# YzM1a0/MuDPT

Measured on AMD Instinct MI355X. Metric: images/sec fwd+bwd ViT-B/16 MuDPT, higher is better.
Workload: dtype bf16; 1 GPU; MuDPT ViT-B/16 fwd+bwd+SGD, batch 256/GPU, 11 class prompts, n_ctx 4, depth 12, synthetic 224x224 N(0,1) images, random-init frozen CLIP (BASELINE configs[1]); global_batch=256, parallelism=dp1

## Files before the change

### mudpt_amd/csrc/gemm_pp.hip

```cpp
#include <hip/hip_ext.h>

#include <type_traits>

#include "kernels.h"

namespace mudpt {

using lptr_t = __attribute__((address_space(3))) void*;

#define VMCNT(n) asm volatile("s_waitcnt vmcnt(" #n ")" ::: "memory")
typedef __attribute__((ext_vector_type(4))) unsigned int u32x4;

template <int N>
__device__ inline void vmcnt() {
    static_assert(N >= 0 && N <= 63, "vmcnt immediate is 6 bits");
    asm volatile("s_waitcnt vmcnt(%0)" ::"n"(N) : "memory");
}

constexpr int EPI_GELU_SPLIT = 100;
constexpr int EPI_GELU_SPLIT8 = 101;
constexpr int EPI_GELU_Q8 = 102;
constexpr int EPI_GELU_BWD_Q8 = 103;

template <typename T, int EPI, bool F8 = false, int ST = 0, int LD = 0, int ABL = 0>
__global__ __launch_bounds__(512) void gemm_pp_kernel(GemmArgs p, int ntn, int ntiles, int rem_half) {
    using elem = typename T::elem;
    using vec8 = typename T::vec8;
    constexpr int STAGE = 65536, BOFF = 32768;
    extern __shared__ __attribute__((aligned(16))) char smem[];

    const int tid = threadIdx.x, lane = tid & 63;
    const int w = __builtin_amdgcn_readfirstlane(tid >> 6);
    const int wr = w >> 2, wc = w & 3;
    const int frow = lane & 15, fq = lane >> 4;

    const int nkt1 = p.K >> 6;
    const int nkt = nkt1 + (p.lo_mode == LO_NONE ? 0 : (F8 ? nkt1 >> 1 : nkt1));
    const int G = gridDim.x;
    const int my_full = rem_half ? ntiles / G : (ntiles - (int)blockIdx.x + G - 1) / G;
    const bool has_half = rem_half && (int)blockIdx.x < 2 * rem_half;
    const int total = (my_full + (has_half ? 1 : 0)) * nkt;

    const auto rsA = __builtin_amdgcn_make_buffer_rsrc(const_cast<void*>(p.A), 0, (int)((size_t)p.M * p.lda * 2 < 0xffffffffull ? (size_t)p.M * p.lda * 2 : 0xffffffffull), 0x00020000);
    const auto rsB = __builtin_amdgcn_make_buffer_rsrc(const_cast<void*>(p.B), 0, (int)((size_t)p.N * p.ldb * 2 < 0xffffffffull ? (size_t)p.N * p.ldb * 2 : 0xffffffffull), 0x00020000);
    const auto rsA2 = __builtin_amdgcn_make_buffer_rsrc(const_cast<void*>(p.A_lo ? p.A_lo : p.A), 0, (int)((size_t)p.M * p.lda * 2 < 0xffffffffull ? (size_t)p.M * p.lda * 2 : 0xffffffffull), 0x00020000);
    const auto rsB2 = __builtin_amdgcn_make_buffer_rsrc(const_cast<void*>(F8 ? p.B8 : p.B), 0, (int)((size_t)p.N * p.ldb * 2 < 0xffffffffull ? (size_t)p.N * p.ldb * 2 : 0xffffffffull), 0x00020000);

    static_assert(EPI == EPI_STORE || EPI == EPI_GELU || EPI == EPI_GELU_SPLIT || EPI == EPI_GELU_SPLIT8 || EPI == EPI_GELU_BWD || EPI == EPI_STORE_F32 ||
                  EPI == EPI_GELU_Q8 || EPI == EPI_GELU_BWD_Q8, "epilogue not built for gemm_pp");
    constexpr bool GELU = (EPI == EPI_GELU || EPI == EPI_GELU_SPLIT || EPI == EPI_GELU_SPLIT8 || EPI == EPI_GELU_Q8);
    constexpr int OOB = (int)0x80000000;
    constexpr bool OUT_F32 = (EPI == EPI_STORE_F32);
    constexpr bool NAT = OUT_F32;
    constexpr int NST = (EPI == EPI_STORE || EPI == EPI_GELU_BWD || EPI == EPI_GELU_BWD_Q8) ? 16 : (EPI == EPI_GELU_SPLIT ? 48 : (EPI == EPI_GELU_SPLIT8 ? 40 : (EPI == EPI_GELU_Q8 ? 24 : 32)));
    const auto rsOut0 = __builtin_amdgcn_make_buffer_rsrc(p.out0, 0, p.M * p.ldo0 * (OUT_F32 ? 4 : (EPI == EPI_GELU_Q8 ? 1 : 2)), 0x00020000);
    const auto rsOut1 = __builtin_amdgcn_make_buffer_rsrc(p.out1, 0, GELU ? p.M * p.ldo1 * 2 : 0, 0x00020000);
    const auto rsOut1Lo = __builtin_amdgcn_make_buffer_rsrc(p.out1_lo, 0, (EPI == EPI_GELU_SPLIT || EPI == EPI_GELU_SPLIT8) ? p.M * p.ldo1 * 2 : 0, 0x00020000);
    const auto rsAux = __builtin_amdgcn_make_buffer_rsrc(const_cast<void*>(p.aux), 0, EPI == EPI_GELU_BWD ? p.M * p.ldaux * 2 : (EPI == EPI_GELU_BWD_Q8 ? p.M * p.ldaux : 0), 0x00020000);
    const auto rsBias = __builtin_amdgcn_make_buffer_rsrc(const_cast<float*>(p.bias), 0, p.bias ? p.N * 4 : 0, 0x00020000);
    bool epi_pending = false;

    int grp[4][2];
#pragma unroll
    for (int q = 0; q < 2; ++q) {
        const int k = 2 * w + q;
        grp[0][q] = k < 8 ? k : k + 8;
        grp[3][q] = k < 8 ? k + 8 : k + 16;
        grp[1][q] = NAT ? (k >> 2) * 8 + (k & 3) : 2 * k;
        grp[2][q] = NAT ? (k >> 2) * 8 + (k & 3) + 4 : 2 * k + 1;
    }
    const int srow = lane >> 3, sslot = lane & 7;
    int lane_off[4][2];
#pragma unroll
    for (int u = 0; u < 4; ++u)
#pragma unroll
        for (int q = 0; q < 2; ++q) {
            const bool isA = (u == 0 || u == 3);
            const int row = grp[u][q] * 8 + srow;
            const int f = (isA || NAT) ? (row & 7) : ((row & 3) | (((row >> 4) & 1) << 2));
            lane_off[u][q] = (row * (isA ? p.lda : p.ldb) + ((sslot ^ f) << 3)) * 2;
        }

    const int gn_knob = (p.flags >> 8) & 0xff;
    const int GN = gn_knob > 0 ? gn_knob : (ntn >= 12 ? 6 : (ntn >= 6 && ntn % 3 == 0 ? 3 : ntn));
    const int ntm = ntiles / ntn;
    auto tile_mn = [&](int tile, int& tm, int& tn) {
        const int tpg = ntm * GN, full = ntn / GN, ng = tile / tpg;
        if (ng < full) {
            const int rem = tile - ng * tpg;
            tm = rem / GN;
            tn = ng * GN + (rem - tm * GN);
        } else {
            const int wl = ntn - full * GN, rem = tile - full * tpg;
            tm = rem / wl;
            tn = full * GN + (rem - tm * wl);
        }
    };
    auto item_tile = [&](int it, int& tm, int& tn, int& h) {
        if (it < my_full) {
            tile_mn(xcd_remap((int)blockIdx.x + it * G, ntiles), tm, tn);
            h = 0;
        } else {
            h = (int)blockIdx.x >= rem_half ? 1 : 0;
            tile_mn(xcd_remap(my_full * G + (int)blockIdx.x - h * rem_half, ntiles), tm, tn);
        }
    };
    int n_kt = 0, n_it = 0, n_baseA = 0, n_baseB = 0, n_soff = 0;
    bool n_second = false;
    bool n_half = false;
    auto set_next_item = [&](int it) {
        int tm, tn, h;
        item_tile(it, tm, tn, h);
        n_half = it >= my_full;
        n_baseA = (tm * 256 + (n_half ? h * 128 - (w >= 4 ? 64 : 0) : 0)) * p.lda * 2;
        n_baseB = tn * 256 * p.ldb * 2;
    };
    auto advance_next = [&]() {
        n_soff += 128;
        if (++n_kt == nkt) {
            n_kt = 0; n_soff = 0; n_second = false;
            if ((++n_it) * nkt < total) set_next_item(n_it);
        } else if (n_kt == nkt1) {
            n_soff = 0; n_second = true;
        }
    };
    auto issue = [&](int u, int stage) {
        if constexpr (ABL & 2) return;
        const bool isA = (u == 0 || u == 3);
        const int base = isA ? n_baseA : n_baseB;
        char* dst = smem + stage * STAGE + (isA ? 0 : BOFF);
#pragma unroll
        for (int q = 0; q < 2; ++q)
            __builtin_amdgcn_raw_ptr_buffer_load_lds(isA ? (n_second ? rsA2 : rsA) : (n_second ? rsB2 : rsB), (lptr_t)(dst + grp[u][q] * 1024), 16, lane_off[u][q] + base, n_soff, 0, 0);
    };

    const int sw = frow & 7;
    const int c0 = (fq ^ sw) << 4;
    const int c8 = ((2 * fq) ^ sw) << 4;
    int ca = c0, cb = c0 ^ 64;
    const int a_base = (wr * 128 + frow) * 128;
    const int b_base = BOFF + (NAT ? wc * 64 + frow : wc * 64 + (frow >> 2) * 16 + (frow & 3)) * 128;
    constexpr int BJ = NAT ? 2048 : 512;

    f32x4 acc[8][4];
#pragma unroll
    for (int i = 0; i < 8; ++i)
#pragma unroll
        for (int j = 0; j < 4; ++j) acc[i][j] = f32x4{0.f, 0.f, 0.f, 0.f};

    if (total > 0) {
        set_next_item(0);
        issue(0, 0); issue(1, 0); issue(2, 0);
        if (!n_half) issue(3, 0);
        advance_next();
    }
    VMCNT(0);
    __builtin_amdgcn_s_barrier();
    if (wr == 1) __builtin_amdgcn_s_barrier();

    typedef __attribute__((ext_vector_type(4))) int i32x4;
    i32x8 af[4], bf[4];
    if constexpr (ABL & 1) {
#pragma unroll
        for (int i = 0; i < 4; ++i) { af[i] = i32x8{lane, 1, 2, 3, 4, 5, 6, 7} * 0x3c003c00; bf[i] = i32x8{7, 6, 5, 4, 3, 2, 1, lane} * 0x3c003c00; }
    }
    auto half = [](const i32x8& v, int ks) -> vec8 {
        return __builtin_bit_cast(vec8, ks ? __builtin_shufflevector(v, v, 4, 5, 6, 7) : __builtin_shufflevector(v, v, 0, 1, 2, 3));
    };
    int c_it = 0;

    auto mfma_quadrant = [&](auto f8tag, int i0, int j0) {
        __builtin_amdgcn_sched_barrier(0);
        __builtin_amdgcn_s_setprio(1);
        if constexpr (decltype(f8tag)::value) {
#pragma unroll
            for (int i = 0; i < 4; ++i)
#pragma unroll
                for (int j = 0; j < 2; ++j)
                    acc[i0 + i][j0 + j] = __builtin_amdgcn_mfma_scale_f32_16x16x128_f8f6f4(bf[j0 + j], af[i], acc[i0 + i][j0 + j], 0, 0, 0, p.b8_scale, 0, LO8_SCALE_E8M0);
        } else {
#pragma unroll
            for (int ks = 0; ks < 2; ++ks)
#pragma unroll
                for (int i = 0; i < 4; ++i)
#pragma unroll
                    for (int j = 0; j < 2; ++j) acc[i0 + i][j0 + j] = T::mfma16(half(bf[j0 + j], ks), half(af[i], ks), acc[i0 + i][j0 + j]);
        }
        __builtin_amdgcn_s_setprio(0);
        __builtin_amdgcn_sched_barrier(0);
    };
    auto read_a = [&](const char* st, int i0) {
        if constexpr (ABL & 1) return;
#pragma unroll
        for (int i = 0; i < 4; ++i)
            af[i] = __builtin_shufflevector(*(const i32x4*)(st + a_base + (i0 + i) * 2048 + ca), *(const i32x4*)(st + a_base + (i0 + i) * 2048 + cb), 0, 1, 2, 3, 4, 5, 6, 7);
    };
    auto read_b = [&](const char* st, int j0) {
        if constexpr (ABL & 1) return;
#pragma unroll
        for (int j = j0; j < j0 + 2; ++j)
            bf[j] = __builtin_shufflevector(*(const i32x4*)(st + b_base + j * BJ + ca), *(const i32x4*)(st + b_base + j * BJ + cb), 0, 1, 2, 3, 4, 5, 6, 7);
    };
    auto epilogue = [&]() {
            int tm, tn, h;
            const bool c_half = c_it >= my_full;
            item_tile(c_it++, tm, tn, h);
            const int ni = c_half ? 4 : 8;
            const int n = tn * 256 + wc * 64 + (NAT ? fq * 4 : fq * 16);
            f32x4 bias4[4];
#pragma unroll
            for (int j = 0; j < 4; ++j)
                bias4[j] = p.bias ? __builtin_bit_cast(f32x4, __builtin_amdgcn_raw_buffer_load_b128(rsBias, (n + (NAT ? 16 : 4) * j) * 4, 0, 0)) : f32x4{0.f, 0.f, 0.f, 0.f};
            const int m_base = tm * 256 + (c_half ? h * 128 + wr * 64 : wr * 128) + frow;
            auto row_off = [&](int i, int ld, int esz, int col) { return (col < p.N ? (m_base * ld + col) * esz : OOB) + i * (16 * ld * esz); };
#pragma unroll
            for (int i = 0; i < 8; ++i)
#pragma unroll
                for (int j = 0; j < 4; ++j) acc[i][j] += bias4[j];
            if constexpr (EPI == EPI_GELU_BWD) {
                vec8 u[8][2];
#pragma unroll
                for (int i = 0; i < 8; ++i) {
                    const int off = i < ni ? row_off(i, p.ldaux, 2, n) : OOB;
                    u[i][0] = __builtin_bit_cast(vec8, __builtin_amdgcn_raw_buffer_load_b128(rsAux, off, 0, LD));
                    u[i][1] = __builtin_bit_cast(vec8, __builtin_amdgcn_raw_buffer_load_b128(rsAux, off, 16, LD));
                }
#pragma unroll
                for (int i = 0; i < 8; ++i)
#pragma unroll
                    for (int j = 0; j < 4; ++j)
#pragma unroll
                        for (int c = 0; c < 4; ++c) acc[i][j][c] *= quick_gelu_grad((float)u[i][j >> 1][4 * (j & 1) + c]);
            }
            if constexpr (EPI == EPI_GELU_BWD_Q8) {
                u32x4 q[8];
#pragma unroll
                for (int i = 0; i < 8; ++i) q[i] = __builtin_amdgcn_raw_buffer_load_b128(rsAux, i < ni ? row_off(i, p.ldaux, 1, n) : OOB, 0, LD);
#pragma unroll
                for (int i = 0; i < 8; ++i)
#pragma unroll
                    for (int j = 0; j < 4; ++j)
#pragma unroll
                        for (int c = 0; c < 4; ++c) acc[i][j][c] *= gelu_grad_from_q8(q[i][j], c);
            }
            __builtin_amdgcn_sched_barrier(0);
#pragma unroll
            for (int i = 0; i < 8; ++i) {
                if (i < ni) {
                if constexpr (OUT_F32) {
#pragma unroll
                    for (int j = 0; j < 4; ++j) __builtin_amdgcn_raw_buffer_store_b128(__builtin_bit_cast(u32x4, acc[i][j]), rsOut0, row_off(i, p.ldo0, 4, n + 16 * j), 0, ST);
                } else {
                    vec8 o0, o1;
                    if constexpr (EPI == EPI_GELU_Q8) {
                        u32x4 q;
#pragma unroll
                        for (int j = 0; j < 4; ++j) q[j] = gelu_grad_q8x4(acc[i][j][0], acc[i][j][1], acc[i][j][2], acc[i][j][3]);
                        __builtin_amdgcn_raw_buffer_store_b128(q, rsOut0, row_off(i, p.ldo0, 1, n), 0, ST);
                    } else {
#pragma unroll
                        for (int c = 0; c < 4; ++c) {
                            o0[c] = round_to<elem>(acc[i][0][c]); o0[4 + c] = round_to<elem>(acc[i][1][c]);
                            o1[c] = round_to<elem>(acc[i][2][c]); o1[4 + c] = round_to<elem>(acc[i][3][c]);
                        }
                        const int off = row_off(i, p.ldo0, 2, n);
                        __builtin_amdgcn_raw_buffer_store_b128(__builtin_bit_cast(u32x4, o0), rsOut0, off, 0, ST);
                        __builtin_amdgcn_raw_buffer_store_b128(__builtin_bit_cast(u32x4, o1), rsOut0, off, 16, ST);
                    }
                    if constexpr (EPI == EPI_GELU || EPI == EPI_GELU_Q8) {
#pragma unroll
                        for (int c = 0; c < 4; ++c) {
                            o0[c] = round_to<elem>(quick_gelu(acc[i][0][c])); o0[4 + c] = round_to<elem>(quick_gelu(acc[i][1][c]));
                            o1[c] = round_to<elem>(quick_gelu(acc[i][2][c])); o1[4 + c] = round_to<elem>(quick_gelu(acc[i][3][c]));
                        }
                        const int off1 = row_off(i, p.ldo1, 2, n);
                        __builtin_amdgcn_raw_buffer_store_b128(__builtin_bit_cast(u32x4, o0), rsOut1, off1, 0, ST);
                        __builtin_amdgcn_raw_buffer_store_b128(__builtin_bit_cast(u32x4, o1), rsOut1, off1, 16, ST);
                    }
                    if constexpr (EPI == EPI_GELU_SPLIT8) {
                        u32x4 l8;
                        float rem[4];
#pragma unroll
                        for (int j = 0; j < 4; ++j) {
#pragma unroll
                            for (int c = 0; c < 4; ++c) {
                                elem hv;
                                rem[c] = split_rem(quick_gelu(acc[i][j][c]), hv);
                                if (j < 2) o0[4 * j + c] = hv; else o1[4 * (j - 2) + c] = hv;
                            }
                            l8[j] = pack_lo8(rem[0], rem[1], rem[2], rem[3]);
                        }
                        const int off1 = row_off(i, p.ldo1, 2, n);
                        __builtin_amdgcn_raw_buffer_store_b128(__builtin_bit_cast(u32x4, o0), rsOut1, off1, 0, ST);
                        __builtin_amdgcn_raw_buffer_store_b128(__builtin_bit_cast(u32x4, o1), rsOut1, off1, 16, ST);
                        __builtin_amdgcn_raw_buffer_store_b128(l8, rsOut1Lo, (n < p.N ? m_base * p.ldo1 * 2 + n : OOB) + i * (32 * p.ldo1), 0, ST);
                    }
                    if constexpr (EPI == EPI_GELU_SPLIT) {
                        vec8 l0, l1;
#pragma unroll
                        for (int c = 0; c < 4; ++c) {
                            elem hv, lv;
                            split_hi_lo(quick_gelu(acc[i][0][c]), hv, lv); o0[c] = hv; l0[c] = lv;
                            split_hi_lo(quick_gelu(acc[i][1][c]), hv, lv); o0[4 + c] = hv; l0[4 + c] = lv;
                            split_hi_lo(quick_gelu(acc[i][2][c]), hv, lv); o1[c] = hv; l1[c] = lv;
                            split_hi_lo(quick_gelu(acc[i][3][c]), hv, lv); o1[4 + c] = hv; l1[4 + c] = lv;
                        }
                        const int off1 = row_off(i, p.ldo1, 2, n);
                        __builtin_amdgcn_raw_buffer_store_b128(__builtin_bit_cast(u32x4, o0), rsOut1, off1, 0, ST);
                        __builtin_amdgcn_raw_buffer_store_b128(__builtin_bit_cast(u32x4, o1), rsOut1, off1, 16, ST);
                        __builtin_amdgcn_raw_buffer_store_b128(__builtin_bit_cast(u32x4, l0), rsOut1Lo, off1, 0, ST);
                        __builtin_amdgcn_raw_buffer_store_b128(__builtin_bit_cast(u32x4, l1), rsOut1Lo, off1, 16, ST);
                    }
                }
                }
#pragma unroll
                for (int j = 0; j < 4; ++j) acc[i][j] = f32x4{0.f, 0.f, 0.f, 0.f};
            }
            epi_pending = true;
    };

    int s = 0;
    auto full_step = [&](auto f8tag) {
        constexpr bool F8S = decltype(f8tag)::value;
        const int cur = s & 1;
        const char* st = smem + cur * STAGE;
        const bool nxt = s + 1 < total;
        ca = F8S ? c8 : c0;
        cb = F8S ? (c8 ^ 16) : (c0 ^ 64);
        read_a(st, 0);
        read_b(st, 0);
        if (nxt) {
            issue(0, cur ^ 1);
            if (epi_pending) vmcnt<NST + 4>(); else vmcnt<4>();
        } else {
            if (epi_pending) vmcnt<NST + 2>(); else vmcnt<2>();
        }
        __builtin_amdgcn_s_barrier();
        mfma_quadrant(f8tag, 0, 0);
        __builtin_amdgcn_s_barrier();
        read_b(st, 2);
        if (nxt) {
            issue(1, cur ^ 1);
            if (epi_pending) vmcnt<NST + 4>(); else vmcnt<4>();
        } else {
            if (epi_pending) vmcnt<NST>(); else vmcnt<0>();
        }
        epi_pending = false;
        __builtin_amdgcn_s_barrier();
        mfma_quadrant(f8tag, 0, 2);
        __builtin_amdgcn_s_barrier();
        read_a(st, 4);
        if (nxt) issue(2, cur ^ 1);
        __builtin_amdgcn_s_barrier();
        mfma_quadrant(f8tag, 4, 2);
        __builtin_amdgcn_s_barrier();
        if (nxt) {
            if (!n_half) { issue(3, cur ^ 1); advance_next(); VMCNT(4); } else { advance_next(); VMCNT(2); }
        }
        __builtin_amdgcn_s_barrier();
        mfma_quadrant(f8tag, 4, 0);
        __builtin_amdgcn_s_barrier();
        ++s;
    };
    auto half_step = [&](auto f8tag) {
        constexpr bool F8S = decltype(f8tag)::value;
        const int cur = s & 1;
        const char* st = smem + cur * STAGE;
        const bool nxt = s + 1 < total;
        ca = F8S ? c8 : c0;
        cb = F8S ? (c8 ^ 16) : (c0 ^ 64);
        read_a(st, 0);
        read_b(st, 0);
        if (nxt) {
            issue(0, cur ^ 1);
            issue(1, cur ^ 1);
            if (epi_pending) vmcnt<NST + 4>(); else vmcnt<4>();
        } else {
            if (epi_pending) vmcnt<NST>(); else vmcnt<0>();
        }
        __builtin_amdgcn_s_barrier();
        mfma_quadrant(f8tag, 0, 0);
        __builtin_amdgcn_s_barrier();
        read_b(st, 2);
        if (nxt) { issue(2, cur ^ 1); advance_next(); VMCNT(2); }
        epi_pending = false;
        __builtin_amdgcn_s_barrier();
        mfma_quadrant(f8tag, 0, 2);
        __builtin_amdgcn_s_barrier();
        ++s;
    };
    const int nkt2 = nkt - nkt1;
    for (int it = 0; it < my_full; ++it) {
        if constexpr (F8) {
            for (int k = 0; k < nkt1; ++k) full_step(std::false_type{});
            for (int k = 0; k < nkt2; ++k) full_step(std::true_type{});
        } else {
            for (int k = 0; k < nkt; ++k) full_step(std::false_type{});
        }
        epilogue();
    }
    if (has_half) {
        if constexpr (F8) {
            for (int k = 0; k < nkt1; ++k) half_step(std::false_type{});
            for (int k = 0; k < nkt2; ++k) half_step(std::true_type{});
        } else {
            for (int k = 0; k < nkt; ++k) half_step(std::false_type{});
        }
        epilogue();
    }
    if (wr == 0) __builtin_amdgcn_s_barrier();
}

template <typename T, int EPI, bool F8 = false, int ST = 0, int LD = 0, int ABL = 0>
static int launch_pp(const GemmArgs& a, hipStream_t s, const GemmOpts& o) {
    constexpr int lds = 2 * 65536;
    constexpr auto kern = gemm_pp_kernel<T, EPI, F8, ST, LD, ABL>;
    const int dev = current_device(), ncu = device_cus(dev);
    if (ncu <= 0) return MUDPT_ERR_HIP;
    if (int e = lds_limit_once<kern>(dev, lds)) return e;
    const int ntm = (a.M + 255) / 256, ntn = (a.N + 255) / 256, ntiles = ntm * ntn;
    int grid = ntiles < ncu ? (2 * ntiles <= ncu ? 2 * ntiles : ntiles) : ncu;
    if (a.flags & 2) grid = ntiles < ncu ? ntiles : ncu;
    const int rem = ntiles % grid, rem_half = (rem > 0 && 2 * rem <= grid && !(a.flags & 2)) ? rem : 0;
    if (o.ev_start && o.ev_stop) {
        hipExtLaunchKernelGGL(kern, dim3(grid), dim3(512), lds, s, o.ev_start, o.ev_stop, 0, a, ntn, ntiles, rem_half);
    } else {
        hipLaunchKernelGGL(kern, dim3(grid), dim3(512), lds, s, a, ntn, ntiles, rem_half);
    }
    HIP_TRY(hipGetLastError());
    return MUDPT_OK;
}

template <typename T>
static int launch_pp_t(int epi, const GemmArgs& a, hipStream_t s, const GemmOpts& o) {
    if constexpr (T::id == DT_F16) {
        if (a.lo_mode == LO_F8) {
            switch (epi) {
                case EPI_STORE: return launch_pp<T, EPI_STORE, true>(a, s, o);
                case EPI_GELU:
                    if (!a.out1_lo) return launch_pp<T, EPI_GELU, true>(a, s, o);
                    return a.out1_lo_mode == LO_F8 ? launch_pp<T, EPI_GELU_SPLIT8, true>(a, s, o) : launch_pp<T, EPI_GELU_SPLIT, true>(a, s, o);
                case EPI_STORE_F32: return launch_pp<T, EPI_STORE_F32, true>(a, s, o);
            }
            set_error("gemm_pp: epilogue %d is not built with the e4m3 second pass", epi);
            return MUDPT_ERR_ARG;
        }
    }
    if constexpr (T::id == DT_BF16) {
        if (epi == EPI_STORE && (a.flags & 0x30)) {
            switch ((a.flags >> 4) & 3) {
                case 1: return launch_pp<T, EPI_STORE, false, 0, 0, 1>(a, s, o);
                case 2: return launch_pp<T, EPI_STORE, false, 0, 0, 2>(a, s, o);
                default: return launch_pp<T, EPI_STORE, false, 0, 0, 3>(a, s, o);
            }
        }
    }
    switch (epi) {
        case EPI_STORE: return launch_pp<T, EPI_STORE>(a, s, o);
        case EPI_GELU:
            if (!a.out1_lo) return a.gelu_q8 ? launch_pp<T, EPI_GELU_Q8>(a, s, o) : launch_pp<T, EPI_GELU>(a, s, o);
            return a.out1_lo_mode == LO_F8 ? launch_pp<T, EPI_GELU_SPLIT8>(a, s, o) : launch_pp<T, EPI_GELU_SPLIT>(a, s, o);
        case EPI_GELU_BWD: return a.gelu_q8 ? launch_pp<T, EPI_GELU_BWD_Q8>(a, s, o) : launch_pp<T, EPI_GELU_BWD>(a, s, o);
        case EPI_STORE_F32: return launch_pp<T, EPI_STORE_F32>(a, s, o);
    }
    set_error("gemm_pp: epilogue %d is not built for the ping-pong kernel", epi);
    return MUDPT_ERR_ARG;
}

int launch_gemm_pp(int dtype, int epi, const GemmArgs& a, hipStream_t s, const GemmOpts& o) {
    ARG_CHECK((size_t)a.M * a.lda * 2 < 0xffffffffull && (size_t)a.N * a.ldb * 2 < 0xffffffffull, "gemm_pp: operand larger than 4 GiB");
    ARG_CHECK(a.lda % 8 == 0 && a.ldb % 8 == 0 && a.ldo0 % 8 == 0, "gemm_pp: strides must be multiples of 8");
    ARG_CHECK(!a.out1_lo || (uintptr_t)a.out1_lo % 16 == 0, "gemm_pp: out1_lo must be 16-byte aligned");
    ARG_CHECK(!a.gelu_q8 || (a.lo_mode == LO_NONE && a.ldo0 % 16 == 0 && a.ldaux % 16 == 0), "gemm_pp: gelu_q8 needs 16-byte row strides and no split operand");
    ARG_CHECK((size_t)a.M * a.ldo0 * (epi == EPI_STORE_F32 ? 4 : 2) < 0x7fffffffull && (size_t)a.M * (size_t)(a.ldo1 > a.ldaux ? a.ldo1 : a.ldaux) * 2 < 0x7fffffffull, "gemm_pp: output larger than 2 GiB");
    if (dtype == DT_BF16) return launch_pp_t<BF16>(epi, a, s, o);
    if (dtype == DT_F16) return launch_pp_t<F16>(epi, a, s, o);
    set_error("gemm: unknown dtype %d", dtype);
    return MUDPT_ERR_ARG;
}

}
```

Before: 10770 images/s.

## Prefetch epilogue bias and GELU-grad codes during last K-step of each tile

Bias vectors and the q8 GELU-gradient codes for the epilogue are now loaded during the final K-step of each tile rather than at the start of the epilogue, so their latency overlaps the last MFMA quadrants. The waitcnt values are adjusted to account for the extra outstanding loads. Loads are also issued unconditionally, using an OOB base once no next tile remains, which removes the nxt branches and their wait variants. This costs extra registers for the prefetched values, and the hand-counted vmcnt values are fragile.

```diff
diff --git a/mudpt_amd/csrc/gemm_pp.hip b/mudpt_amd/csrc/gemm_pp.hip
--- a/mudpt_amd/csrc/gemm_pp.hip
+++ b/mudpt_amd/csrc/gemm_pp.hip
@@ -15,6 +15,20 @@
 __device__ inline void vmcnt() {
     static_assert(N >= 0 && N <= 63, "vmcnt immediate is 6 bits");
     asm volatile("s_waitcnt vmcnt(%0)" ::"n"(N) : "memory");
+}
+
+template <int N, int NQ>
+__device__ inline void vmcnt_pf(int pf) {
+    if (pf == 0) vmcnt<N>();
+    else if (NQ == 0 || pf == 4) vmcnt<N + 4>();
+    else if (pf == NQ) vmcnt<N + NQ>();
+    else vmcnt<N + NQ + 4>();
+}
+
+template <int N>
+__device__ inline void vmcnt_seen() {
+    static_assert(N >= 0 && N <= 15, "low four bits only");
+    __builtin_amdgcn_s_waitcnt(0x0f70 | N);
 }
 
 constexpr int EPI_GELU_SPLIT = 100;
@@ -58,6 +72,14 @@
     const auto rsOut1Lo = __builtin_amdgcn_make_buffer_rsrc(p.out1_lo, 0, (EPI == EPI_GELU_SPLIT || EPI == EPI_GELU_SPLIT8) ? p.M * p.ldo1 * 2 : 0, 0x00020000);
     const auto rsAux = __builtin_amdgcn_make_buffer_rsrc(const_cast<void*>(p.aux), 0, EPI == EPI_GELU_BWD ? p.M * p.ldaux * 2 : (EPI == EPI_GELU_BWD_Q8 ? p.M * p.ldaux : 0), 0x00020000);
     const auto rsBias = __builtin_amdgcn_make_buffer_rsrc(const_cast<float*>(p.bias), 0, p.bias ? p.N * 4 : 0, 0x00020000);
+    constexpr int NQ = EPI == EPI_GELU_BWD_Q8 ? 8 : 0;
+    constexpr bool PFB = !F8 && EPI != EPI_GELU_BWD_Q8;
+    const int npf = (PFB && p.bias ? 4 : 0) + NQ;
+    static_assert(NST + 4 + 4 + NQ <= 63, "the counted waits of a tile's last K-step");
+    f32x4 bias_pf[4];
+#pragma unroll
+    for (int j = 0; j < 4; ++j) bias_pf[j] = f32x4{0.f, 0.f, 0.f, 0.f};
+    u32x4 codes[NQ ? NQ : 1];
     bool epi_pending = false;
 
     int grp[4][2];
@@ -108,18 +130,25 @@
     int n_kt = 0, n_it = 0, n_baseA = 0, n_baseB = 0, n_soff = 0;
     bool n_second = false;
     bool n_half = false;
+    int n_row = 0, n_col = 0;
+    int e_row = 0, e_col = 0;
+    bool e_half = false;
     auto set_next_item = [&](int it) {
         int tm, tn, h;
         item_tile(it, tm, tn, h);
         n_half = it >= my_full;
         n_baseA = (tm * 256 + (n_half ? h * 128 - (w >= 4 ? 64 : 0) : 0)) * p.lda * 2;
         n_baseB = tn * 256 * p.ldb * 2;
+        n_row = tm * 256 + (n_half ? h * 128 : 0);
+        n_col = tn * 256;
     };
     auto advance_next = [&]() {
         n_soff += 128;
         if (++n_kt == nkt) {
             n_kt = 0; n_soff = 0; n_second = false;
+            e_row = n_row; e_col = n_col; e_half = n_half;
             if ((++n_it) * nkt < total) set_next_item(n_it);
+            else n_baseA = n_baseB = OOB;
         } else if (n_kt == nkt1) {
             n_soff = 0; n_second = true;
         }
@@ -132,6 +161,20 @@
 #pragma unroll
         for (int q = 0; q < 2; ++q)
             __builtin_amdgcn_raw_ptr_buffer_load_lds(isA ? (n_second ? rsA2 : rsA) : (n_second ? rsB2 : rsB), (lptr_t)(dst + grp[u][q] * 1024), 16, lane_off[u][q] + base, n_soff, 0, 0);
+    };
+
+    auto epi_prefetch = [&]() {
+        const int n = e_col + wc * 64 + (NAT ? fq * 4 : fq * 16);
+        if (PFB && p.bias) {
+#pragma unroll
+            for (int j = 0; j < 4; ++j) bias_pf[j] = __builtin_bit_cast(f32x4, __builtin_amdgcn_raw_buffer_load_b128(rsBias, (n + (NAT ? 16 : 4) * j) * 4, 0, 0));
+        }
+        if constexpr (NQ) {
+            const int off0 = n < p.N ? (e_row + (e_half ? wr * 64 : wr * 128) + frow) * p.ldaux + n : OOB, ni = e_half ? 4 : 8;
+#pragma unroll
+            for (int i = 0; i < NQ; ++i) codes[i] = __builtin_amdgcn_raw_buffer_load_b128(rsAux, i < ni ? off0 + i * (16 * p.ldaux) : OOB, 0, LD);
+        }
+        __builtin_amdgcn_sched_barrier(0);
     };
 
     const int sw = frow & 7;
@@ -207,16 +250,27 @@
             item_tile(c_it++, tm, tn, h);
             const int ni = c_half ? 4 : 8;
             const int n = tn * 256 + wc * 64 + (NAT ? fq * 4 : fq * 16);
-            f32x4 bias4[4];
-#pragma unroll
-            for (int j = 0; j < 4; ++j)
-                bias4[j] = p.bias ? __builtin_bit_cast(f32x4, __builtin_amdgcn_raw_buffer_load_b128(rsBias, (n + (NAT ? 16 : 4) * j) * 4, 0, 0)) : f32x4{0.f, 0.f, 0.f, 0.f};
             const int m_base = tm * 256 + (c_half ? h * 128 + wr * 64 : wr * 128) + frow;
             auto row_off = [&](int i, int ld, int esz, int col) { return (col < p.N ? (m_base * ld + col) * esz : OOB) + i * (16 * ld * esz); };
-#pragma unroll
-            for (int i = 0; i < 8; ++i)
-#pragma unroll
-                for (int j = 0; j < 4; ++j) acc[i][j] += bias4[j];
+            auto add_bias = [&](const f32x4 (&b)[4]) {
+#pragma unroll
+                for (int i = 0; i < 8; ++i)
+#pragma unroll
+                    for (int j = 0; j < 4; ++j) acc[i][j] += b[j];
+            };
+            if constexpr (PFB) {
+                add_bias(bias_pf);
+            } else {
+                f32x4 bias4[4];
+#pragma unroll
+                for (int j = 0; j < 4; ++j) bias4[j] = f32x4{0.f, 0.f, 0.f, 0.f};
+                if (p.bias) {
+#pragma unroll
+                    for (int j = 0; j < 4; ++j) bias4[j] = __builtin_bit_cast(f32x4, __builtin_amdgcn_raw_buffer_load_b128(rsBias, (n + (NAT ? 16 : 4) * j) * 4, 0, 0));
+                    vmcnt_seen<0>();
+                }
+                add_bias(bias4);
+            }
             if constexpr (EPI == EPI_GELU_BWD) {
                 vec8 u[8][2];
 #pragma unroll
@@ -233,15 +287,12 @@
                         for (int c = 0; c < 4; ++c) acc[i][j][c] *= quick_gelu_grad((float)u[i][j >> 1][4 * (j & 1) + c]);
             }
             if constexpr (EPI == EPI_GELU_BWD_Q8) {
-                u32x4 q[8];
-#pragma unroll
-                for (int i = 0; i < 8; ++i) q[i] = __builtin_amdgcn_raw_buffer_load_b128(rsAux, i < ni ? row_off(i, p.ldaux, 1, n) : OOB, 0, LD);
 #pragma unroll
                 for (int i = 0; i < 8; ++i)
 #pragma unroll
                     for (int j = 0; j < 4; ++j)
 #pragma unroll
-                        for (int c = 0; c < 4; ++c) acc[i][j][c] *= gelu_grad_from_q8(q[i][j], c);
+                        for (int c = 0; c < 4; ++c) acc[i][j][c] *= gelu_grad_from_q8(codes[i][j], c);
             }
             __builtin_amdgcn_sched_barrier(0);
 #pragma unroll
@@ -320,69 +371,68 @@
     };
 
     int s = 0;
-    auto full_step = [&](auto f8tag) {
+    auto full_step = [&](auto f8tag, bool last) {
         constexpr bool F8S = decltype(f8tag)::value;
         const int cur = s & 1;
         const char* st = smem + cur * STAGE;
         const bool nxt = s + 1 < total;
+        const int pf = last ? npf : 0;
         ca = F8S ? c8 : c0;
         cb = F8S ? (c8 ^ 16) : (c0 ^ 64);
         read_a(st, 0);
         read_b(st, 0);
-        if (nxt) {
-            issue(0, cur ^ 1);
-            if (epi_pending) vmcnt<NST + 4>(); else vmcnt<4>();
+        if (last) epi_prefetch();
+        issue(0, cur ^ 1);
+        if (epi_pending) vmcnt_pf<NST + 4, NQ>(pf); else vmcnt_pf<4, NQ>(pf);
+        __builtin_amdgcn_s_barrier();
+        mfma_quadrant(f8tag, 0, 0);
+        __builtin_amdgcn_s_barrier();
+        read_b(st, 2);
+        issue(1, cur ^ 1);
+        if (epi_pending) vmcnt_pf<NST + 4, NQ>(pf); else vmcnt_pf<4, NQ>(pf);
+        epi_pending = false;
+        __builtin_amdgcn_s_barrier();
+        mfma_quadrant(f8tag, 0, 2);
+        __builtin_amdgcn_s_barrier();
+        read_a(st, 4);
+        issue(2, cur ^ 1);
+        __builtin_amdgcn_s_barrier();
+        mfma_quadrant(f8tag, 4, 2);
+        __builtin_amdgcn_s_barrier();
+        if (!n_half) {
+            issue(3, cur ^ 1);
+            if (nxt) advance_next();
+            vmcnt_seen<4>();
         } else {
-            if (epi_pending) vmcnt<NST + 2>(); else vmcnt<2>();
-        }
-        __builtin_amdgcn_s_barrier();
-        mfma_quadrant(f8tag, 0, 0);
-        __builtin_amdgcn_s_barrier();
-        read_b(st, 2);
-        if (nxt) {
-            issue(1, cur ^ 1);
-            if (epi_pending) vmcnt<NST + 4>(); else vmcnt<4>();
-        } else {
-            if (epi_pending) vmcnt<NST>(); else vmcnt<0>();
-        }
-        epi_pending = false;
-        __builtin_amdgcn_s_barrier();
-        mfma_quadrant(f8tag, 0, 2);
-        __builtin_amdgcn_s_barrier();
-        read_a(st, 4);
-        if (nxt) issue(2, cur ^ 1);
-        __builtin_amdgcn_s_barrier();
-        mfma_quadrant(f8tag, 4, 2);
-        __builtin_amdgcn_s_barrier();
-        if (nxt) {
-            if (!n_half) { issue(3, cur ^ 1); advance_next(); VMCNT(4); } else { advance_next(); VMCNT(2); }
+            if (nxt) advance_next();
+            vmcnt_seen<2>();
         }
         __builtin_amdgcn_s_barrier();
         mfma_quadrant(f8tag, 4, 0);
         __builtin_amdgcn_s_barrier();
         ++s;
     };
-    auto half_step = [&](auto f8tag) {
+    auto half_step = [&](auto f8tag, bool last) {
         constexpr bool F8S = decltype(f8tag)::value;
         const int cur = s & 1;
         const char* st = smem + cur * STAGE;
         const bool nxt = s + 1 < total;
+        const int pf = last ? npf : 0;
         ca = F8S ? c8 : c0;
         cb = F8S ? (c8 ^ 16) : (c0 ^ 64);
         read_a(st, 0);
         read_b(st, 0);
-        if (nxt) {
-            issue(0, cur ^ 1);
-            issue(1, cur ^ 1);
-            if (epi_pending) vmcnt<NST + 4>(); else vmcnt<4>();
-        } else {
-            if (epi_pending) vmcnt<NST>(); else vmcnt<0>();
-        }
+        if (last) epi_prefetch();
+        issue(0, cur ^ 1);
+        issue(1, cur ^ 1);
+        if (epi_pending) vmcnt_pf<NST + 4, NQ>(pf); else vmcnt_pf<4, NQ>(pf);
         __builtin_amdgcn_s_barrier();
         mfma_quadrant(f8tag, 0, 0);
         __builtin_amdgcn_s_barrier();
         read_b(st, 2);
-        if (nxt) { issue(2, cur ^ 1); advance_next(); VMCNT(2); }
+        issue(2, cur ^ 1);
+        if (nxt) advance_next();
+        vmcnt_seen<2>();
         epi_pending = false;
         __builtin_amdgcn_s_barrier();
         mfma_quadrant(f8tag, 0, 2);
@@ -392,22 +442,23 @@
     const int nkt2 = nkt - nkt1;
     for (int it = 0; it < my_full; ++it) {
         if constexpr (F8) {
-            for (int k = 0; k < nkt1; ++k) full_step(std::false_type{});
-            for (int k = 0; k < nkt2; ++k) full_step(std::true_type{});
+            for (int k = 0; k < nkt1; ++k) full_step(std::false_type{}, nkt2 == 0 && k == nkt1 - 1);
+            for (int k = 0; k < nkt2; ++k) full_step(std::true_type{}, k == nkt2 - 1);
         } else {
-            for (int k = 0; k < nkt; ++k) full_step(std::false_type{});
+            for (int k = 0; k < nkt; ++k) full_step(std::false_type{}, k == nkt - 1);
         }
         epilogue();
     }
     if (has_half) {
         if constexpr (F8) {
-            for (int k = 0; k < nkt1; ++k) half_step(std::false_type{});
-            for (int k = 0; k < nkt2; ++k) half_step(std::true_type{});
+            for (int k = 0; k < nkt1; ++k) half_step(std::false_type{}, nkt2 == 0 && k == nkt1 - 1);
+            for (int k = 0; k < nkt2; ++k) half_step(std::true_type{}, k == nkt2 - 1);
         } else {
-            for (int k = 0; k < nkt; ++k) half_step(std::false_type{});
+            for (int k = 0; k < nkt; ++k) half_step(std::false_type{}, k == nkt - 1);
         }
         epilogue();
     }
+    VMCNT(0);
     if (wr == 0) __builtin_amdgcn_s_barrier();
 }
 
```

New measurement: 10660 images/s. 1.0% lower.
